# daniloceano/LorenzCycleToolkit

Measured on NVIDIA B200. Metric: LEC timesteps/s (all terms), 0.25°×37-lvl ERA5 shape; % of HBM roofline, higher is better.
Workload: dtype f32

## Files before the change

### lorenzcycletoolkit_b200/csrc/lec_row_body.inc

```
#if LEC_BODY_EDGE == 2
    const bool edge_iter = (it == 0) || (it == niter - 1) || (VEC == 1);
#else
    constexpr bool edge_iter = (LEC_BODY_EDGE != 0);
#endif
    if (!edge_iter || lane_on) {
    CT wgv[VEC], cav[VEC], ccv[VEC];
#pragma unroll
    for (int e = 0; e < VEC; ++e) { wgv[e] = CT(1); cav[e] = cxa_u; ccv[e] = cxc_u; }
    if constexpr (LONW >= 1) {
      if constexpr (sizeof(CT) == 4) {
        float w4[VEC];
        LEC_TAB_LOAD(LEC_TAB_WL + col, w4);
#pragma unroll
        for (int e = 0; e < VEC; ++e) wgv[e] = CT(w4[e]);
        if constexpr (LONW == 2) {
          float a4[VEC], c4[VEC];
          LEC_TAB_LOAD(LEC_TAB_CXA + col, a4);
          LEC_TAB_LOAD(LEC_TAB_CXC + col, c4);
#pragma unroll
          for (int e = 0; e < VEC; ++e) { cav[e] = rc.fx * CT(a4[e]); ccv[e] = rc.fx * CT(c4[e]); }
        }
      } else {
#pragma unroll
        for (int e = 0; e < VEC; ++e) {
// ... 48 lines not shown
        const P tc = P::make(CT(Tc[e]), CT(Tc[e + 1]));
        const P dtdt = pfma(P::bcast(rc.ct_m), P::make(CT(Tm[e]), CT(Tm[e + 1])) - tc,
                            pfma(P::bcast(rc.ct_p), P::make(CT(Tp[e]), CT(Tp[e + 1])) - tc, P::bcast(rc.ct_s) * tc));
        const P dTx = pfma(P::make(cav[e], cav[e + 1]), P::make(CT(tlv[e]), CT(tlv[e + 1])) - tc,
                           P::make(ccv[e], ccv[e + 1]) * (P::make(CT(trv[e]), CT(trv[e + 1])) - tc));
        const P dTy = pfma(P::bcast(rc.cy_m), P::make(CT(Tjm[e]), CT(Tjm[e + 1])) - tc,
                           P::bcast(rc.cy_p) * (P::make(CT(Tjp[e]), CT(Tjp[e + 1])) - tc));
        const P Ss = pfma(P::bcast(rc.s_m), P::make(CT(Tkm[e]), CT(Tkm[e + 1])) - tc,
                          pfma(P::bcast(rc.s_p), P::make(CT(Tkp[e]), CT(Tkp[e + 1])) - tc, P::bcast(rc.s_s) * tc));
        const P u = P::make(CT(U[e]), CT(U[e + 1])), v = P::make(CT(V[e]), CT(V[e + 1])),
                om = P::make(CT(W[e]), CT(W[e + 1]));
        q[h] = pfma(u, dTx, pfma(v, dTy, pfma(om, Ss, dtdt)));
        a[h] = tc - P::bcast(cshT); b[h] = u - P::bcast(cshU); cv[h] = v - P::bcast(cshV); w[h] = om - P::bcast(cshW);
        f[h] = P::make(CT(F[e]), CT(F[e + 1])) - P::bcast(cshF);
        if (masked) {
          const CT z = CT(0);
          a[h] = P::make(inb(e) ? a[h].lo() : z, inb(e + 1) ? a[h].hi() : z);
          b[h] = P::make(inb(e) ? b[h].lo() : z, inb(e + 1) ? b[h].hi() : z);
          cv[h] = P::make(inb(e) ? cv[h].lo() : z, inb(e + 1) ? cv[h].hi() : z);
          w[h] = P::make(inb(e) ? w[h].lo() : z, inb(e + 1) ? w[h].hi() : z);
          f[h] = P::make(inb(e) ? f[h].lo() : z, inb(e + 1) ? f[h].hi() : z);
          q[h] = P::make(inb(e) ? q[h].lo() : z, inb(e + 1) ? q[h].hi() : z);
        }
        Wa[h] = a[h]; Wb[h] = b[h]; Wc[h] = cv[h]; Ww[h] = w[h]; Wf[h] = f[h]; Wq[h] = q[h];
        if (weighted) {
          const P wg = P::make(wgv[e], wgv[e + 1]);
          Wa[h] = wg * a[h]; Wb[h] = wg * b[h]; Wc[h] = wg * cv[h]; Ww[h] = wg * w[h]; Wf[h] = wg * f[h]; Wq[h] = wg * q[h];
        }
        pbb[h] = Wb[h] * b[h]; pcc[h] = Wc[h] * cv[h]; pca[h] = Wc[h] * a[h]; pwa[h] = Ww[h] * a[h];
      }
      if constexpr (NPAIR == 2) {
        auto lin = [](P x0, P x1) { const P t = x0 + x1; return t.lo() + t.hi(); };
        auto prd = [](P x0, P y0, P x1, P y1) { const P t = pfma(x1, y1, x0 * y0); return t.lo() + t.hi(); };
        lec_lin_add<CT, COMP>(S[R_A], Cc[R_A], lin(Wa[0], Wa[1])); lec_lin_add<CT, COMP>(S[R_B], Cc[R_B], lin(Wb[0], Wb[1]));
        lec_lin_add<CT, COMP>(S[R_C], Cc[R_C], lin(Wc[0], Wc[1])); lec_lin_add<CT, COMP>(S[R_W], Cc[R_W], lin(Ww[0], Ww[1]));
        lec_lin_add<CT, COMP>(S[R_F], Cc[R_F], lin(Wf[0], Wf[1])); lec_lin_add<CT, COMP>(S[R_Q], Cc[R_Q], lin(Wq[0], Wq[1]));
        S[R_AA] += prd(Wa[0], a[0], Wa[1], a[1]); S[R_BB] += lin(pbb[0], pbb[1]); S[R_CC] += lin(pcc[0], pcc[1]);
        S[R_BC] += prd(Wb[0], cv[0], Wb[1], cv[1]); S[R_CA] += lin(pca[0], pca[1]); S[R_WA] += lin(pwa[0], pwa[1]);
        S[R_WB] += prd(Ww[0], b[0], Ww[1], b[1]); S[R_WC] += prd(Ww[0], cv[0], Ww[1], cv[1]);
        S[R_WF] += prd(Ww[0], f[0], Ww[1], f[1]); S[R_QA] += prd(Wa[0], q[0], Wa[1], q[1]);
        S[R_CAA] += prd(pca[0], a[0], pca[1], a[1]); S[R_WAA] += prd(pwa[0], a[0], pwa[1], a[1]);
        S[R_BBC] += prd(pbb[0], cv[0], pbb[1], cv[1]); S[R_CCC] += prd(pcc[0], cv[0], pcc[1], cv[1]);
        S[R_BBW] += prd(pbb[0], w[0], pbb[1], w[1]); S[R_CCW] += prd(pcc[0], w[0], pcc[1], w[1]);
      } else {
#pragma unroll
        for (int h = 0; h < NPAIR; ++h) {
          accumulate_pp<CT, COMP>(S, Cc, Wa[h].lo(), Wb[h].lo(), Wc[h].lo(), Ww[h].lo(), Wf[h].lo(), Wq[h].lo(), a[h].lo(), b[h].lo(),
                            cv[h].lo(), w[h].lo(), f[h].lo(), q[h].lo(), pbb[h].lo(), pcc[h].lo(), pca[h].lo(), pwa[h].lo());
          accumulate_pp<CT, COMP>(S, Cc, Wa[h].hi(), Wb[h].hi(), Wc[h].hi(), Ww[h].hi(), Wf[h].hi(), Wq[h].hi(), a[h].hi(), b[h].hi(),
                            cv[h].hi(), w[h].hi(), f[h].hi(), q[h].hi(), pbb[h].hi(), pcc[h].hi(), pca[h].hi(), pwa[h].hi());
        }
      }
    } else {
#pragma unroll
      for (int e = 0; e < VEC; ++e) {
        const CT tc = CT(Tc[e]);
        const CT dtdt = rc.ct_m * (CT(Tm[e]) - tc) + rc.ct_p * (CT(Tp[e]) - tc) + rc.ct_s * tc;
        const CT dTx = cav[e] * (CT(tlv[e]) - tc) + ccv[e] * (CT(trv[e]) - tc);
        const CT dTy = rc.cy_m * (CT(Tjm[e]) - tc) + rc.cy_p * (CT(Tjp[e]) - tc);
        const CT Ss = rc.s_m * (CT(Tkm[e]) - tc) + rc.s_p * (CT(Tkp[e]) - tc) + rc.s_s * tc;
        const CT u = CT(U[e]), v = CT(V[e]), om = CT(W[e]);
        CT q = dtdt + u * dTx + v * dTy + om * Ss;
        CT a = tc - cshT, b = u - cshU, cv = v - cshV, w = om - cshW, f = CT(F[e]) - cshF;
        if (masked && !inb(e)) { q = CT(0); a = CT(0); b = CT(0); cv = CT(0); w = CT(0); f = CT(0); }
        const CT wg = wgv[e];
        accumulate_s<CT, COMP>(S, Cc, wg * a, wg * b, wg * cv, wg * w, wg * f, wg * q, a, b, cv, w, f, q);
      }
    }
    }
```

### lorenzcycletoolkit_b200/csrc/lec_row_moments.cuh

```cuda
#pragma once
#include "lec_common.cuh"
#include "lec_packed.cuh"

namespace lec {

#ifndef LEC_ROWS_PER_CTA
#define LEC_ROWS_PER_CTA 2
#endif
constexpr int kRowsPerCta = LEC_ROWS_PER_CTA;
constexpr int kRowThreads = kRowsPerCta * 32;

struct FastDiv {
  unsigned mul;
  unsigned shr;
  unsigned d;
  static FastDiv make(unsigned d) {
    FastDiv f;
    unsigned L = 0;
    while ((1ull << L) < d) ++L;
    f.mul = (unsigned)(((1ull << (31 + L)) / d) + 1ull);
    f.shr = 31 + L;
    f.d = d;
    return f;
  }
// ... 25 lines not shown
  const unsigned long long a0 = reinterpret_cast<unsigned long long>(p) + (unsigned long long)lo_byte;
  const unsigned long long a1 = reinterpret_cast<unsigned long long>(p) + (unsigned long long)hi_byte;
  const unsigned long long lo = (a0 + 15ULL) & ~15ULL, hi = a1 & ~15ULL;
  if (hi <= lo) return;
  const unsigned n = unsigned(hi - lo);
  asm volatile("cp.async.bulk.prefetch.L2.global [%0], %1;" ::"l"(lo), "r"(n) : "memory");
}

#ifdef LEC_NO_STREAM
#define __ldcs __ldg
#endif
template <typename FT, int VEC> struct VecLoad;
template <> struct VecLoad<float, 4> {
  static __device__ __forceinline__ void ld(const float* p, float (&v)[4]) {
    float4 t = __ldg(reinterpret_cast<const float4*>(p)); v[0] = t.x; v[1] = t.y; v[2] = t.z; v[3] = t.w; }
  static __device__ __forceinline__ void ld_stream(const float* p, float (&v)[4]) {
    float4 t = __ldcs(reinterpret_cast<const float4*>(p)); v[0] = t.x; v[1] = t.y; v[2] = t.z; v[3] = t.w; }
};
template <> struct VecLoad<double, 2> {
  static __device__ __forceinline__ void ld(const double* p, double (&v)[2]) {
    double2 t = __ldg(reinterpret_cast<const double2*>(p)); v[0] = t.x; v[1] = t.y; }
  static __device__ __forceinline__ void ld_stream(const double* p, double (&v)[2]) {
    double2 t = __ldcs(reinterpret_cast<const double2*>(p)); v[0] = t.x; v[1] = t.y; }
};
template <typename FT> struct VecLoad<FT, 1> {
  static __device__ __forceinline__ void ld(const FT* p, FT (&v)[1]) { v[0] = __ldg(p); }
  static __device__ __forceinline__ void ld_stream(const FT* p, FT (&v)[1]) { v[0] = __ldcs(p); }
};

__device__ __forceinline__ double shfl_xor_f64(double v, int m) {
  return __shfl_xor_sync(0xffffffffu, v, m);
}

template <int N>
__device__ __forceinline__ double butterfly_reduce(double (&v)[N], int lane) {
  static_assert(N <= 32, "at most one value per lane");
  double a[32];
#pragma unroll
  for (int i = 0; i < 32; ++i) a[i] = (i < N) ? v[i] : 0.0;
  int n = 32;
#pragma unroll
  for (int bit = 16; bit >= 1; bit >>= 1) {
    n >>= 1;
    const bool hi = (lane & bit) != 0;
#pragma unroll
    for (int i = 0; i < n; ++i) {
      const int live = (N + (32 / (2 * n)) - 1) / (32 / (2 * n));
      if (2 * i < live) {
        const double keep = hi ? a[2 * i + 1] : a[2 * i];
        const double send = hi ? a[2 * i] : a[2 * i + 1];
        a[i] = keep + shfl_xor_f64(send, bit);
      } else {
        a[i] = 0.0;
      }
    }
  }
  return a[0];
}

__device__ __forceinline__ int bitrev5(int x) {
  return ((x & 1) << 4) | ((x & 2) << 2) | (x & 4) | ((x & 8) >> 2) | ((x & 16) >> 4);
}

template <typename CT>
struct RowCoefS {
  CT ct_m, ct_p, ct_s;
  CT cy_m, cy_p;
  CT s_m, s_p, s_s;
  CT fx;
};

constexpr int R_NLIN = 6;

template <typename CT, bool COMP>
__device__ __forceinline__ void lec_lin_add(CT& s, CT& c, CT x) {
  if constexpr (sizeof(CT) == 4 && COMP) {
    const CT t = s + x;
    c += x - (t - s);
    s = t;
  } else {
    s += x;
  }
}

template <typename CT, bool COMP>
__device__ __forceinline__ void accumulate_s(CT (&S)[R_NSUM], CT (&Cc)[R_NLIN], CT Wa, CT Wb, CT Wc, CT Ww, CT Wf, CT Wq,
                                           CT a, CT b, CT c, CT w, CT f, CT q) {
  lec_lin_add<CT, COMP>(S[R_A], Cc[R_A], Wa); lec_lin_add<CT, COMP>(S[R_B], Cc[R_B], Wb); lec_lin_add<CT, COMP>(S[R_C], Cc[R_C], Wc);
  lec_lin_add<CT, COMP>(S[R_W], Cc[R_W], Ww); lec_lin_add<CT, COMP>(S[R_F], Cc[R_F], Wf); lec_lin_add<CT, COMP>(S[R_Q], Cc[R_Q], Wq);
// ... 18 lines not shown
}

template <typename CT, int LONW>
struct RowSetup {
  RowCoefS<CT> rc;
  CT cxa_u, cxc_u, cxW, cxE, wW, wE;
  double fxd;
  __device__ __forceinline__ void init(const RowParams& p, const StepDev* __restrict__ st, int j, int k, int j0, int j1) {
    if constexpr (sizeof(CT) == 4) {
      rc.ct_m = st->f_ct_m; rc.ct_p = st->f_ct_p; rc.ct_s = st->f_ct_s;
      rc.cy_m = (j == j0) ? 0.f : (j == j1) ? -st->f_cyN : __ldg(p.g.cya32 + j);
      rc.cy_p = (j == j1) ? 0.f : (j == j0) ? st->f_cyS : __ldg(p.g.cyc32 + j);
      rc.s_m = __ldg(p.g.sm32 + k); rc.s_p = __ldg(p.g.sp32 + k); rc.s_s = __ldg(p.g.ss32 + k);
      rc.fx = __ldg(p.g.fxj32 + j);
      fxd = 0.0;
      cxa_u = rc.fx * p.g.cxa_u32; cxc_u = rc.fx * p.g.cxc_u32;
      cxW = rc.fx * st->f_cxW; cxE = rc.fx * st->f_cxE;
      wW = (LONW == 0) ? st->f_wWn : st->f_wW; wE = (LONW == 0) ? st->f_wEn : st->f_wE;
    } else {
      rc.ct_m = st->ct_m; rc.ct_p = st->ct_p; rc.ct_s = st->ct_s;
      rc.cy_m = (j == j0) ? 0.0 : (j == j1) ? -st->cyN : p.g.cya[j];
      rc.cy_p = (j == j1) ? 0.0 : (j == j0) ? st->cyS : p.g.cyc[j];
      rc.s_m = p.g.sm[k]; rc.s_p = p.g.sp[k]; rc.s_s = p.g.ss[k];
      fxd = p.g.fxj[j];
      rc.fx = fxd;
      cxa_u = fxd * p.g.cxa_u; cxc_u = fxd * p.g.cxc_u;
      cxW = fxd * st->cxW; cxE = fxd * st->cxE;
      const double wnorm = (LONW == 0) ? 1.0 / p.g.wl_u : 1.0;
      wW = st->wW * wnorm; wE = st->wE * wnorm;
    }
  }
};

#ifndef LEC_ROW_MIN_CTAS
#define LEC_ROW_MIN_CTAS (512 / kRowThreads)
#endif
template <typename FT, typename CT, int VEC, int LONW, bool COMP>
__global__ void __launch_bounds__(kRowThreads, sizeof(CT) == 8 ? (LEC_ROW_MIN_CTAS * 3) / 4 : COMP ? (LEC_ROW_MIN_CTAS * 3) / 4 : LEC_ROW_MIN_CTAS)
lec_row_moments_kernel(const RowParams p) {
  const int warp = threadIdx.x >> 5, lane = threadIdx.x & 31;
  const unsigned bid = blockIdx.x;
  unsigned ujt, uk, us;
  const unsigned q1 = p.dv_tiles.divmod(bid, ujt);
  const unsigned q2 = p.dv_lev.divmod(q1, uk);
  const int band = int(p.dv_steps.divmod(q2, us));
  const int jt = int(ujt), k = int(uk), s = int(us);

  const StepDev* __restrict__ st = p.steps + s;
  const int i0 = st->i0, i1 = st->i1, j0 = st->j0, j1 = st->j1;
  const int jrel = (band * p.tiles_per_band + jt) * kRowsPerCta + warp;
  if (jrel > j1 - j0) return;
  const int j = j0 + jrel;
  const int nlon = p.g.nlon, nlat = p.g.nlat, nlev = p.g.nlev;

  const long long plane = (long long)nlat * nlon;
  const long long row_c = ((long long)st->slot * nlev + k) * plane + (long long)j * nlon;
  const FT* __restrict__ Tc_row = static_cast<const FT*>(p.field[0]) + row_c;
  const FT* __restrict__ U_row = static_cast<const FT*>(p.field[1]) + row_c;
  const FT* __restrict__ V_row = static_cast<const FT*>(p.field[2]) + row_c;
  const FT* __restrict__ W_row = static_cast<const FT*>(p.field[3]) + row_c;
  const FT* __restrict__ F_row = static_cast<const FT*>(p.field[4]) + row_c;
  const int d_m = int((long long)(st->slot_m - st->slot) * p.slot_stride);
  const int d_p = int((long long)(st->slot_p - st->slot) * p.slot_stride);
  const int d_km = (k > 0) ? -int(plane) : 0, d_kp = (k < nlev - 1) ? int(plane) : 0;
  const int d_jm = (j > j0) ? -nlon : 0, d_jp = (j < j1) ? nlon : 0;

// ... 17 lines not shown
#pragma unroll
  for (int n = 0; n < R_NSUM; ++n) S[n] = CT(0);
#pragma unroll
  for (int n = 0; n < R_NLIN; ++n) Cc[n] = CT(0);

  double* __restrict__ rec = p.rec + (((long long)s * nlev + k) * p.max_ny + jrel) * LEC_NREC;

  const int c0 = i0 / VEC, c1 = i1 / VEC;
  const int niter = (c1 - c0 + 32) / 32;

  auto at = [](const FT* base, int idx) -> const FT* {
    unsigned long long a;
    asm("mad.wide.s32 %0, %1, %2, %3;" : "=l"(a) : "r"(idx), "r"((int)sizeof(FT)), "l"(base));
    return reinterpret_cast<const FT*>(a);
  };
  {
    const int it = 0;
#define LEC_BODY_EDGE 1
#include "lec_row_iter_direct.inc"
#undef LEC_BODY_EDGE
  }
  for (int it = 1; it < niter - 1; ++it) {
#define LEC_BODY_EDGE 0
#include "lec_row_iter_direct.inc"
#undef LEC_BODY_EDGE
  }
  if (niter > 1) {
    const int it = niter - 1;
#define LEC_BODY_EDGE 1
#include "lec_row_iter_direct.inc"
#undef LEC_BODY_EDGE
  }

  double Sd[R_NSUM];
#pragma unroll
  for (int n = 0; n < R_NSUM; ++n) Sd[n] = double(S[n]);
  if constexpr (sizeof(CT) == 4 && COMP) {
#pragma unroll
    for (int n = 0; n < R_NLIN; ++n) Sd[n] += double(Cc[n]);
  }
  double tot = butterfly_reduce<R_NSUM>(Sd, lane);
  if (LONW == 0) tot *= p.g.wl_u;
  const int idx = bitrev5(lane);
  if (idx < R_NSUM) rec[idx] = tot;
  if (lane == 1) {
    rec[R_SH_T] = double(shT); rec[R_SH_U] = double(shU); rec[R_SH_V] = double(shV);
    rec[R_SH_W] = double(shW); rec[R_SH_F] = double(shF);
  }
}

}
```

### lorenzcycletoolkit_b200/csrc/lec_row_narrow.cuh

```cuda
#pragma once
#include "lec_common.cuh"
#include "lec_packed.cuh"
#include "lec_row_moments.cuh"

namespace lec {

constexpr int kNarrowWarps = 1;
constexpr int kNarrowThreads = kNarrowWarps * 32;

template <int N, int G>
__device__ __forceinline__ void butterfly_reduce_seg(const double (&v)[N], int gl, double (&out)[(N + G - 1) / G]) {
  constexpr int NP = ((N + G - 1) / G) * G;
  double a[NP];
#pragma unroll
  for (int i = 0; i < NP; ++i) a[i] = (i < N) ? v[i] : 0.0;
  int n = NP;
#pragma unroll
  for (int bit = G / 2; bit >= 1; bit >>= 1) {
    n >>= 1;
    const bool hi = (gl & bit) != 0;
#pragma unroll
    for (int i = 0; i < n; ++i) {
      const double keep = hi ? a[2 * i + 1] : a[2 * i];
      const double send = hi ? a[2 * i] : a[2 * i + 1];
      a[i] = keep + __shfl_xor_sync(0xffffffffu, send, bit);
    }
  }
#pragma unroll
  for (int m = 0; m < (N + G - 1) / G; ++m) out[m] = a[m];
}

template <int G>
__device__ __forceinline__ int bitrev_group(int gl) {
  int r = 0;
#pragma unroll
  for (int b = 1, o = G / 2; b < G; b <<= 1, o >>= 1) r |= (gl & b) ? o : 0;
  return r;
}

template <typename FT, typename CT, int VEC, int LONW, int G, bool COMP>
__global__ void __launch_bounds__(kNarrowThreads, (sizeof(CT) == 8 ? 384 : 512) / kNarrowThreads)
lec_row_moments_narrow_kernel(const RowParams p) {
  constexpr int RPW = 32 / G;
  const int warp = threadIdx.x >> 5, lane31 = threadIdx.x & 31;
  const int lane = lane31 & (G - 1);
  const int wr = lane31 / G;
  const unsigned bid = blockIdx.x;
  unsigned ujt, uk, us;
  const unsigned q1 = p.dv_tiles.divmod(bid, ujt);
  const unsigned q2 = p.dv_lev.divmod(q1, uk);
  const int band = int(p.dv_steps.divmod(q2, us));
  const int jt = int(ujt), k = int(uk), s = int(us);

  const StepDev* __restrict__ st = p.steps + s;
  const int i0 = st->i0, i1 = st->i1, j0 = st->j0, j1 = st->j1;
  const int jrel_first = ((band * p.tiles_per_band + jt) * kNarrowWarps + warp) * RPW;
  if (jrel_first > j1 - j0) return;
  const bool row_on = jrel_first + wr <= j1 - j0;
  const int jrel = min(jrel_first + wr, j1 - j0);
  const int j = j0 + jrel;
  const int nlon = p.g.nlon, nlat = p.g.nlat, nlev = p.g.nlev;

// ... 26 lines not shown
  const bool box_aligned = (i0 % VEC == 0) && ((i1 + 1) % VEC == 0);

  const FT shT = __ldg(Tc_row + i0), shU = __ldg(U_row + i0), shV = __ldg(V_row + i0),
           shW = __ldg(W_row + i0), shF = __ldg(F_row + i0);
  const CT cshT = CT(shT), cshU = CT(shU), cshV = CT(shV), cshW = CT(shW), cshF = CT(shF);

  CT S[R_NSUM], Cc[R_NLIN];
#pragma unroll
  for (int n = 0; n < R_NSUM; ++n) S[n] = CT(0);
#pragma unroll
  for (int n = 0; n < R_NLIN; ++n) Cc[n] = CT(0);
  double* __restrict__ rec = p.rec + (((long long)s * nlev + k) * p.max_ny + jrel) * LEC_NREC;

  const int c0 = i0 / VEC, c1 = i1 / VEC;
  const int niter = (c1 - c0 + G) / G;
  {
    const int it = 0;
#define LEC_BODY_EDGE 1
#include "lec_row_iter_narrow.inc"
#undef LEC_BODY_EDGE
  }
  for (int it = 1; it < niter - 1; ++it) {
#define LEC_BODY_EDGE 0
#include "lec_row_iter_narrow.inc"
#undef LEC_BODY_EDGE
  }
  if (niter > 1) {
    const int it = niter - 1;
#define LEC_BODY_EDGE 1
#include "lec_row_iter_narrow.inc"
#undef LEC_BODY_EDGE
  }

  double Sd[R_NSUM];
#pragma unroll
  for (int n = 0; n < R_NSUM; ++n) Sd[n] = double(S[n]);
  if constexpr (sizeof(CT) == 4 && COMP) {
#pragma unroll
    for (int n = 0; n < R_NLIN; ++n) Sd[n] += double(Cc[n]);
  }
  constexpr int NOUT = (R_NSUM + G - 1) / G;
  double tot[NOUT];
  butterfly_reduce_seg<R_NSUM, G>(Sd, lane, tot);
  if (row_on) {
    const int r = bitrev_group<G>(lane);
#pragma unroll
    for (int m = 0; m < NOUT; ++m) {
      const int idx = r + m * G;
      if (idx < R_NSUM) rec[idx] = (LONW == 0) ? tot[m] * p.g.wl_u : tot[m];
    }
    if (lane == 1) {
      rec[R_SH_T] = double(shT); rec[R_SH_U] = double(shU); rec[R_SH_V] = double(shV);
      rec[R_SH_W] = double(shW); rec[R_SH_F] = double(shF);
    }
  }
}

}
```

### lorenzcycletoolkit_b200/csrc/lec_row_tile.cuh

```cuda
#pragma once
#include <cuda.h>

#include "lec_common.cuh"
#include "lec_packed.cuh"
#include "lec_row_moments.cuh"
#include "lec_row_narrow.cuh"

namespace lec {

struct alignas(64) TmaMaps {
  CUtensorMap t_halo;
  CUtensorMap t_plain;
  CUtensorMap u, v, w, f;
};

template <typename FT, int R, int NSTG, int GL = 32>
struct TileGeom {
  static constexpr int VEC = 16 / sizeof(FT);
  static constexpr int RPW = 32 / GL;
  static constexpr int ROWS = R * RPW;
  static constexpr int C = GL * VEC;
  static constexpr int HP = C + 2 * VEC;
  static constexpr int halo_bytes = (ROWS + 2) * HP * sizeof(FT);
  static constexpr int halo_bytes_pad = (halo_bytes + 127) / 128 * 128;
  static constexpr int tile_bytes = ROWS * C * sizeof(FT);
  static constexpr int stage_bytes = halo_bytes_pad + 8 * tile_bytes;
  static constexpr int smem_bytes = NSTG * stage_bytes + 128;
  static constexpr int threads = (R + 1) * 32;
  static __host__ __device__ constexpr int tx_bytes(int rows) { return ((rows + 2) * HP + 8 * rows * C) * (int)sizeof(FT); }
};

__device__ __forceinline__ unsigned smem_u32(const void* p) { return (unsigned)__cvta_generic_to_shared(p); }
__device__ __forceinline__ void mbar_init(unsigned bar, int count) {
  asm volatile("mbarrier.init.shared::cta.b64 [%0], %1;" ::"r"(bar), "r"(count) : "memory");
}
__device__ __forceinline__ void mbar_expect_tx(unsigned bar, unsigned bytes) {
  asm volatile("mbarrier.arrive.expect_tx.shared::cta.b64 _, [%0], %1;" ::"r"(bar), "r"(bytes) : "memory");
}
__device__ __forceinline__ void mbar_arrive(unsigned bar) {
  asm volatile("mbarrier.arrive.shared::cta.b64 _, [%0];" ::"r"(bar) : "memory");
}
__device__ __forceinline__ bool mbar_try_wait(unsigned bar, unsigned parity) {
  unsigned ok;
  asm volatile(
      "{\n .reg .pred p;\n mbarrier.try_wait.parity.shared::cta.b64 p, [%1], %2;\n selp.u32 %0, 1, 0, p;\n}"
      : "=r"(ok) : "r"(bar), "r"(parity) : "memory");
  return ok != 0;
}
__device__ __forceinline__ void mbar_wait(unsigned bar, unsigned parity) {
  while (!mbar_try_wait(bar, parity)) {}
}
template <int OFF>
__device__ __forceinline__ void mbar_arrive_off(unsigned bar) {
  asm volatile("mbarrier.arrive.shared::cta.b64 _, [%0+%1];" ::"r"(bar), "n"(OFF) : "memory");
}
__device__ __forceinline__ unsigned long long l2_policy_evict_first() {
  unsigned long long pol;
  asm volatile("createpolicy.fractional.L2::evict_first.b64 %0, 1.0;" : "=l"(pol));
  return pol;
}
// ... 13 lines not shown

template <typename FT, int VEC>
__device__ __forceinline__ void lds_vec(unsigned a, FT (&v)[VEC]) {
  if constexpr (sizeof(FT) == 4) {
    asm volatile("ld.shared.v4.f32 {%0, %1, %2, %3}, [%4];" : "=f"(v[0]), "=f"(v[1]), "=f"(v[2]), "=f"(v[3]) : "r"(a));
  } else {
    asm volatile("ld.shared.v2.f64 {%0, %1}, [%2];" : "=d"(v[0]), "=d"(v[1]) : "r"(a));
  }
}
__device__ __forceinline__ float lds_one(unsigned a, float) {
  float v; asm volatile("ld.shared.f32 %0, [%1];" : "=f"(v) : "r"(a)); return v;
}
__device__ __forceinline__ double lds_one(unsigned a, double) {
  double v; asm volatile("ld.shared.f64 %0, [%1];" : "=d"(v) : "r"(a)); return v;
}

template <bool SHARED, int VEC>
__device__ __forceinline__ void tab_load(const float* ptr, float (&v)[VEC]) {
  if constexpr (SHARED && VEC == 4) {
    const float4 t = *reinterpret_cast<const float4*>(ptr); v[0] = t.x; v[1] = t.y; v[2] = t.z; v[3] = t.w;
  } else {
    VecLoad<float, VEC>::ld(ptr, v);
  }
}

template <bool SHARED, int VEC>
__device__ __forceinline__ void tab_load_tile(const float* ptr, unsigned saddr, float (&v)[VEC]) {
  if constexpr (SHARED && VEC == 4) {
    asm volatile("ld.shared.v4.f32 {%0, %1, %2, %3}, [%4];" : "=f"(v[0]), "=f"(v[1]), "=f"(v[2]), "=f"(v[3]) : "r"(saddr));
  } else {
    VecLoad<float, VEC>::ld(ptr, v);
  }
}

struct TileId { int band, s, k, jt; };
__device__ __forceinline__ TileId decode_tile(unsigned id, const RowParams& p) {
  TileId t;
  unsigned jt, k, s;
  const unsigned a = p.dv_tiles.divmod(id, jt);
  const unsigned b = p.dv_lev.divmod(a, k);
  t.band = int(p.dv_steps.divmod(b, s));
  t.jt = int(jt); t.k = int(k); t.s = int(s);
  return t;
}

template <typename FT, typename CT, int LONW, int R, int NSTG, bool COMP, bool TABS, int GL = 32, int MINB = 1>
__global__ void __launch_bounds__((R + 1) * 32, MINB)
lec_row_moments_tile_kernel(const __grid_constant__ TmaMaps maps, const RowParams p) {
  using G = TileGeom<FT, R, NSTG, GL>;
  constexpr int VEC = G::VEC, C = G::C, HP = G::HP, RPW = G::RPW;
  const int trows = (GL == 32) ? R : p.tile_rows;
  extern __shared__ __align__(1024) unsigned char smem[];
  unsigned long long* bars = reinterpret_cast<unsigned long long*>(smem + NSTG * G::stage_bytes);
  const unsigned full0 = smem_u32(bars), empty0 = smem_u32(bars + NSTG);
  const int warp = threadIdx.x >> 5, lane = threadIdx.x & 31;

  if (threadIdx.x == 0) {
    for (int i = 0; i < NSTG; ++i) { mbar_init(full0 + 8 * i, 1); mbar_init(empty0 + 8 * i, R); }
    asm volatile("fence.mbarrier_init.release.cluster;" ::: "memory");
  }
  const float* wl_tab = p.g.wl32;
  if constexpr (TABS) {
    float* wl_s = reinterpret_cast<float*>(smem + G::smem_bytes);
    for (int i = threadIdx.x; i < p.g.nlon; i += blockDim.x) wl_s[i] = __ldg(p.g.wl32 + i);
    wl_tab = wl_s;
  }
  __syncthreads();

  const int nlev = p.g.nlev;

  if (warp == R) {
    if (lane == 0) {
      int stg = 0;
      unsigned phase = 0;
      const unsigned long long pol_stream = l2_policy_evict_first();
      for (unsigned id = blockIdx.x; id < (unsigned)p.grid; id += gridDim.x) {
        const TileId t = decode_tile(id, p);
        const StepDev* __restrict__ st = p.steps + t.s;
        const int jr = (t.band * p.tiles_per_band + t.jt) * trows;
        if (jr > st->j1 - st->j0) continue;
        const int c0 = st->i0 / VEC, c1 = st->i1 / VEC;
        const int nch = (c1 - c0 + GL) / GL;
        const unsigned tx = (unsigned)G::tx_bytes(trows);
        const unsigned tile_b = (unsigned)(trows * C * (int)sizeof(FT));
        const int jt0 = st->j0 + jr;
        const int k = t.k, km = k > 0 ? k - 1 : k, kp = k < nlev - 1 ? k + 1 : k;
        const int slot = st->slot, slot_m = st->slot_m, slot_p = st->slot_p;
        int col = c0 * VEC;
        for (int ch = 0; ch < nch; ++ch, col += C) {
          mbar_wait(empty0 + 8 * stg, phase ^ 1);
          const unsigned fb = full0 + 8 * stg;
          if (p.prefetch_mode & 2) {
            mbar_arrive(fb);
            if (++stg == NSTG) { stg = 0; phase ^= 1; }
            continue;
          }
          mbar_expect_tx(fb, tx);
          const unsigned base = smem_u32(smem) + (unsigned)stg * G::stage_bytes;
          tma_load_4d(base, &maps.t_halo, fb, col - VEC, jt0 - 1, k, slot);
          unsigned d = base + G::halo_bytes_pad;
          if (p.prefetch_mode & 8) {
            tma_load_4d_hint(d, &maps.u, fb, col, jt0, k, slot, pol_stream); d += tile_b;
            tma_load_4d_hint(d, &maps.v, fb, col, jt0, k, slot, pol_stream); d += tile_b;
            tma_load_4d_hint(d, &maps.w, fb, col, jt0, k, slot, pol_stream); d += tile_b;
            tma_load_4d_hint(d, &maps.f, fb, col, jt0, k, slot, pol_stream); d += tile_b;
          } else {
            tma_load_4d(d, &maps.u, fb, col, jt0, k, slot); d += tile_b;
            tma_load_4d(d, &maps.v, fb, col, jt0, k, slot); d += tile_b;
            tma_load_4d(d, &maps.w, fb, col, jt0, k, slot); d += tile_b;
            tma_load_4d(d, &maps.f, fb, col, jt0, k, slot); d += tile_b;
          }
          tma_load_4d(d, &maps.t_plain, fb, col, jt0, k, slot_p); d += tile_b;
          tma_load_4d(d, &maps.t_plain, fb, col, jt0, k, slot_m); d += tile_b;
          tma_load_4d(d, &maps.t_plain, fb, col, jt0, km, slot); d += tile_b;
          tma_load_4d(d, &maps.t_plain, fb, col, jt0, kp, slot);
          if (++stg == NSTG) { stg = 0; phase ^= 1; }
        }
      }
    }
    return;
  }

  const unsigned sbase0 = smem_u32(smem);
  const int gl = lane & (GL - 1);
  const int rowt = warp * RPW + lane / GL;
  const unsigned off_hc = (unsigned)(((rowt + 1) * HP + VEC + gl * VEC) * sizeof(FT));
  const unsigned off_t = (unsigned)(G::halo_bytes_pad + (rowt * C + gl * VEC) * sizeof(FT));
  const unsigned kTile = (unsigned)(trows * C * (int)sizeof(FT));
  unsigned sb = sbase0, fb = full0;
  int stg = 0;
  unsigned phase = 0;
  [[maybe_unused]] unsigned wl_s32 = 0;
  if constexpr (TABS) wl_s32 = smem_u32(smem + G::smem_bytes);
  for (unsigned id = blockIdx.x; id < (unsigned)p.grid; id += gridDim.x) {
    const TileId t = decode_tile(id, p);
    const StepDev* __restrict__ st = p.steps + t.s;
    const int i0 = st->i0, i1 = st->i1, j0 = st->j0, j1 = st->j1;
    const int jrel0 = (t.band * p.tiles_per_band + t.jt) * trows;
    if (jrel0 > j1 - j0) continue;
    const bool warp_on = (warp * RPW < trows) && (jrel0 + warp * RPW <= j1 - j0) && !(p.prefetch_mode & 4);
    const bool row_on = warp_on && (rowt < trows) && (jrel0 + rowt <= j1 - j0);
    const int jrel = row_on ? jrel0 + rowt : j1 - j0;
    const int j = j0 + jrel;
    const int k = t.k;
    const int c0 = i0 / VEC, c1 = i1 / VEC;
    const int niter = (c1 - c0 + GL) / GL;

    RowSetup<CT, LONW> rs;
    rs.init(p, st, j, k, j0, j1);
    const RowCoefS<CT>& rc = rs.rc;
    const CT cxa_u = rs.cxa_u, cxc_u = rs.cxc_u, cxW = rs.cxW, cxE = rs.cxE, wW = rs.wW, wE = rs.wE;
    [[maybe_unused]] const double fxd = rs.fxd;
    const bool box_aligned = (i0 % VEC == 0) && ((i1 + 1) % VEC == 0);
    const unsigned off_hm = (j > j0) ? off_hc - (unsigned)(HP * sizeof(FT)) : off_hc;
    const unsigned off_hp = (j < j1) ? off_hc + (unsigned)(HP * sizeof(FT)) : off_hc;

    FT shT = FT(0), shU = FT(0), shV = FT(0), shW = FT(0), shF = FT(0);
    CT cshT = CT(0), cshU = CT(0), cshV = CT(0), cshW = CT(0), cshF = CT(0);
    CT S[R_NSUM], Cc[R_NLIN];
#pragma unroll
    for (int n = 0; n < R_NSUM; ++n) S[n] = CT(0);
#pragma unroll
    for (int n = 0; n < R_NLIN; ++n) Cc[n] = CT(0);
    double* __restrict__ rec = p.rec + (((long long)t.s * nlev + k) * p.max_ny + jrel) * LEC_NREC;


    {
      const int it = 0;
#define LEC_BODY_EDGE 1
#define LEC_ITER_FIRST 1
#include "lec_row_iter_tile.inc"
#undef LEC_ITER_FIRST
#undef LEC_BODY_EDGE
    }
    for (int it = 1; it < niter - 1; ++it) {
#define LEC_BODY_EDGE 0
#define LEC_ITER_FIRST 0
#include "lec_row_iter_tile.inc"
#undef LEC_ITER_FIRST
#undef LEC_BODY_EDGE
    }
    if (niter > 1) {
      const int it = niter - 1;
#define LEC_BODY_EDGE 1
#define LEC_ITER_FIRST 0
#include "lec_row_iter_tile.inc"
#undef LEC_ITER_FIRST
#undef LEC_BODY_EDGE
    }

    if (warp_on) {
      double Sd[R_NSUM];
#pragma unroll
      for (int n = 0; n < R_NSUM; ++n) Sd[n] = double(S[n]);
      if constexpr (sizeof(CT) == 4 && COMP) {
#pragma unroll
        for (int n = 0; n < R_NLIN; ++n) Sd[n] += double(Cc[n]);
      }
      if constexpr (GL == 32) {
        double tot = butterfly_reduce<R_NSUM>(Sd, lane);
        if (LONW == 0) tot *= p.g.wl_u;
        const int idx = bitrev5(lane);
        if (idx < R_NSUM) rec[idx] = tot;
      } else {
        constexpr int NOUT = (R_NSUM + GL - 1) / GL;
        double tot[NOUT];
        butterfly_reduce_seg<R_NSUM, GL>(Sd, gl, tot);
        if (row_on) {
          const int r = bitrev_group<GL>(gl);
#pragma unroll
          for (int m = 0; m < NOUT; ++m) {
            const int idx = r + m * GL;
            if (idx < R_NSUM) rec[idx] = (LONW == 0) ? tot[m] * p.g.wl_u : tot[m];
          }
        }
      }
      if (row_on && gl == 1) {
        rec[R_SH_T] = double(shT); rec[R_SH_U] = double(shU); rec[R_SH_V] = double(shV);
        rec[R_SH_W] = double(shW); rec[R_SH_F] = double(shF);
      }
    }
  }
}

}
```

Baseline: 6423.

## Move per-tile row setup to producer warp and pair float accumulations

The TMA producer warp now computes each tile's per-row setup (coefficients, halo offsets, record pointers) into a double-buffered shared-memory header guarded by new mbarriers, so consumer warps no longer redo decode and RowSetup work at every tile. Separately, the inner accumulation updates pairs of sums with paired float adds. The warp reductions also do their first butterfly step in float before widening to double when compensation is off. The costs are extra shared memory, additional barrier handshakes, and float-precision loss in the first reduction step.

After: 6515 (median of 6 runs). 1.01x the previous value.

```diff
diff --git a/lorenzcycletoolkit_b200/csrc/lec_row_body.inc b/lorenzcycletoolkit_b200/csrc/lec_row_body.inc
--- a/lorenzcycletoolkit_b200/csrc/lec_row_body.inc
+++ b/lorenzcycletoolkit_b200/csrc/lec_row_body.inc
@@ -104,16 +104,28 @@
       if constexpr (NPAIR == 2) {
         auto lin = [](P x0, P x1) { const P t = x0 + x1; return t.lo() + t.hi(); };
         auto prd = [](P x0, P y0, P x1, P y1) { const P t = pfma(x1, y1, x0 * y0); return t.lo() + t.hi(); };
-        lec_lin_add<CT, COMP>(S[R_A], Cc[R_A], lin(Wa[0], Wa[1])); lec_lin_add<CT, COMP>(S[R_B], Cc[R_B], lin(Wb[0], Wb[1]));
-        lec_lin_add<CT, COMP>(S[R_C], Cc[R_C], lin(Wc[0], Wc[1])); lec_lin_add<CT, COMP>(S[R_W], Cc[R_W], lin(Ww[0], Ww[1]));
-        lec_lin_add<CT, COMP>(S[R_F], Cc[R_F], lin(Wf[0], Wf[1])); lec_lin_add<CT, COMP>(S[R_Q], Cc[R_Q], lin(Wq[0], Wq[1]));
-        S[R_AA] += prd(Wa[0], a[0], Wa[1], a[1]); S[R_BB] += lin(pbb[0], pbb[1]); S[R_CC] += lin(pcc[0], pcc[1]);
-        S[R_BC] += prd(Wb[0], cv[0], Wb[1], cv[1]); S[R_CA] += lin(pca[0], pca[1]); S[R_WA] += lin(pwa[0], pwa[1]);
-        S[R_WB] += prd(Ww[0], b[0], Ww[1], b[1]); S[R_WC] += prd(Ww[0], cv[0], Ww[1], cv[1]);
-        S[R_WF] += prd(Ww[0], f[0], Ww[1], f[1]); S[R_QA] += prd(Wa[0], q[0], Wa[1], q[1]);
-        S[R_CAA] += prd(pca[0], a[0], pca[1], a[1]); S[R_WAA] += prd(pwa[0], a[0], pwa[1], a[1]);
-        S[R_BBC] += prd(pbb[0], cv[0], pbb[1], cv[1]); S[R_CCC] += prd(pcc[0], cv[0], pcc[1], cv[1]);
-        S[R_BBW] += prd(pbb[0], w[0], pbb[1], w[1]); S[R_CCW] += prd(pcc[0], w[0], pcc[1], w[1]);
+        auto acc = [&](int n, CT x, CT y) {
+          if constexpr (COMP) {
+            if (n < R_NLIN) {
+              lec_lin_add<CT, COMP>(S[n], Cc[n], x); lec_lin_add<CT, COMP>(S[n + 1], Cc[n + 1], y);
+              return;
+            }
+          }
+          const P t = P::make(S[n], S[n + 1]) + P::make(x, y);
+          S[n] = t.lo(); S[n + 1] = t.hi();
+        };
+        static_assert(R_B == R_A + 1 && R_W == R_C + 1 && R_Q == R_F + 1 && R_NLIN % 2 == 0 && R_NSUM % 2 == 0, "sums pair up");
+        acc(R_A, lin(Wa[0], Wa[1]), lin(Wb[0], Wb[1]));
+        acc(R_C, lin(Wc[0], Wc[1]), lin(Ww[0], Ww[1]));
+        acc(R_F, lin(Wf[0], Wf[1]), lin(Wq[0], Wq[1]));
+        acc(R_AA, prd(Wa[0], a[0], Wa[1], a[1]), lin(pbb[0], pbb[1]));
+        acc(R_CC, lin(pcc[0], pcc[1]), prd(Wb[0], cv[0], Wb[1], cv[1]));
+        acc(R_CA, lin(pca[0], pca[1]), lin(pwa[0], pwa[1]));
+        acc(R_WB, prd(Ww[0], b[0], Ww[1], b[1]), prd(Ww[0], cv[0], Ww[1], cv[1]));
+        acc(R_WF, prd(Ww[0], f[0], Ww[1], f[1]), prd(Wa[0], q[0], Wa[1], q[1]));
+        acc(R_CAA, prd(pca[0], a[0], pca[1], a[1]), prd(pwa[0], a[0], pwa[1], a[1]));
+        acc(R_BBC, prd(pbb[0], cv[0], pbb[1], cv[1]), prd(pcc[0], cv[0], pcc[1], cv[1]));
+        acc(R_BBW, prd(pbb[0], w[0], pbb[1], w[1]), prd(pcc[0], w[0], pcc[1], w[1]));
       } else {
 #pragma unroll
         for (int h = 0; h < NPAIR; ++h) {
diff --git a/lorenzcycletoolkit_b200/csrc/lec_row_moments.cuh b/lorenzcycletoolkit_b200/csrc/lec_row_moments.cuh
--- a/lorenzcycletoolkit_b200/csrc/lec_row_moments.cuh
+++ b/lorenzcycletoolkit_b200/csrc/lec_row_moments.cuh
@@ -81,20 +81,14 @@
   return __shfl_xor_sync(0xffffffffu, v, m);
 }
 
-template <int N>
-__device__ __forceinline__ double butterfly_reduce(double (&v)[N], int lane) {
-  static_assert(N <= 32, "at most one value per lane");
-  double a[32];
-#pragma unroll
-  for (int i = 0; i < 32; ++i) a[i] = (i < N) ? v[i] : 0.0;
-  int n = 32;
-#pragma unroll
-  for (int bit = 16; bit >= 1; bit >>= 1) {
-    n >>= 1;
+template <int N, int BIT>
+__device__ __forceinline__ void butterfly_steps(double (&a)[32], int lane) {
+#pragma unroll
+  for (int bit = BIT; bit >= 1; bit >>= 1) {
     const bool hi = (lane & bit) != 0;
 #pragma unroll
-    for (int i = 0; i < n; ++i) {
-      const int live = (N + (32 / (2 * n)) - 1) / (32 / (2 * n));
+    for (int i = 0; i < bit; ++i) {
+      const int live = (N + (16 / bit) - 1) / (16 / bit);
       if (2 * i < live) {
         const double keep = hi ? a[2 * i + 1] : a[2 * i];
         const double send = hi ? a[2 * i] : a[2 * i + 1];
@@ -104,6 +98,34 @@
       }
     }
   }
+}
+
+template <int N>
+__device__ __forceinline__ double butterfly_reduce(double (&v)[N], int lane) {
+  static_assert(N <= 32, "at most one value per lane");
+  double a[32];
+#pragma unroll
+  for (int i = 0; i < 32; ++i) a[i] = (i < N) ? v[i] : 0.0;
+  butterfly_steps<N, 16>(a, lane);
+  return a[0];
+}
+
+template <int N>
+__device__ __forceinline__ double butterfly_reduce(const float (&v)[N], int lane) {
+  static_assert(N <= 32, "at most one value per lane");
+  double a[32];
+  const bool hi = (lane & 16) != 0;
+#pragma unroll
+  for (int i = 0; i < 16; ++i) {
+    if (2 * i < N) {
+      const float v0 = v[2 * i], v1 = (2 * i + 1 < N) ? v[2 * i + 1] : 0.f;
+      const float keep = hi ? v1 : v0, send = hi ? v0 : v1;
+      a[i] = double(keep) + double(__shfl_xor_sync(0xffffffffu, send, 16));
+    } else {
+      a[i] = 0.0;
+    }
+  }
+  butterfly_steps<N, 8>(a, lane);
   return a[0];
 }
 
@@ -188,6 +210,22 @@
   }
 };
 
+template <typename CT, bool COMP>
+__device__ __forceinline__ double row_reduce(const CT (&S)[R_NSUM], const CT (&Cc)[R_NLIN], int lane) {
+  if constexpr (sizeof(CT) == 4 && !COMP) {
+    return butterfly_reduce<R_NSUM>(S, lane);
+  } else {
+    double Sd[R_NSUM];
+#pragma unroll
+    for (int n = 0; n < R_NSUM; ++n) Sd[n] = double(S[n]);
+    if constexpr (sizeof(CT) == 4) {
+#pragma unroll
+      for (int n = 0; n < R_NLIN; ++n) Sd[n] += double(Cc[n]);
+    }
+    return butterfly_reduce<R_NSUM>(Sd, lane);
+  }
+}
+
 #ifndef LEC_ROW_MIN_CTAS
 #define LEC_ROW_MIN_CTAS (512 / kRowThreads)
 #endif
@@ -271,14 +309,7 @@
 #undef LEC_BODY_EDGE
   }
 
-  double Sd[R_NSUM];
-#pragma unroll
-  for (int n = 0; n < R_NSUM; ++n) Sd[n] = double(S[n]);
-  if constexpr (sizeof(CT) == 4 && COMP) {
-#pragma unroll
-    for (int n = 0; n < R_NLIN; ++n) Sd[n] += double(Cc[n]);
-  }
-  double tot = butterfly_reduce<R_NSUM>(Sd, lane);
+  double tot = row_reduce<CT, COMP>(S, Cc, lane);
   if (LONW == 0) tot *= p.g.wl_u;
   const int idx = bitrev5(lane);
   if (idx < R_NSUM) rec[idx] = tot;
diff --git a/lorenzcycletoolkit_b200/csrc/lec_row_narrow.cuh b/lorenzcycletoolkit_b200/csrc/lec_row_narrow.cuh
--- a/lorenzcycletoolkit_b200/csrc/lec_row_narrow.cuh
+++ b/lorenzcycletoolkit_b200/csrc/lec_row_narrow.cuh
@@ -8,15 +8,22 @@
 constexpr int kNarrowWarps = 1;
 constexpr int kNarrowThreads = kNarrowWarps * 32;
 
-template <int N, int G>
-__device__ __forceinline__ void butterfly_reduce_seg(const double (&v)[N], int gl, double (&out)[(N + G - 1) / G]) {
+template <int N, int G, typename T>
+__device__ __forceinline__ void butterfly_reduce_seg(const T (&v)[N], int gl, double (&out)[(N + G - 1) / G]) {
   constexpr int NP = ((N + G - 1) / G) * G;
-  double a[NP];
+  double a[NP / 2];
+  {
+    const bool hi = (gl & (G / 2)) != 0;
 #pragma unroll
-  for (int i = 0; i < NP; ++i) a[i] = (i < N) ? v[i] : 0.0;
-  int n = NP;
+    for (int i = 0; i < NP / 2; ++i) {
+      const T v0 = (2 * i < N) ? v[2 * i] : T(0), v1 = (2 * i + 1 < N) ? v[2 * i + 1] : T(0);
+      const T keep = hi ? v1 : v0, send = hi ? v0 : v1;
+      a[i] = double(keep) + double(__shfl_xor_sync(0xffffffffu, send, G / 2));
+    }
+  }
+  int n = NP / 2;
 #pragma unroll
-  for (int bit = G / 2; bit >= 1; bit >>= 1) {
+  for (int bit = G / 4; bit >= 1; bit >>= 1) {
     n >>= 1;
     const bool hi = (gl & bit) != 0;
 #pragma unroll
@@ -28,6 +35,23 @@
   }
 #pragma unroll
   for (int m = 0; m < (N + G - 1) / G; ++m) out[m] = a[m];
+}
+
+template <typename CT, bool COMP, int G>
+__device__ __forceinline__ void row_reduce_seg(const CT (&S)[R_NSUM], const CT (&Cc)[R_NLIN], int gl,
+                                               double (&out)[(R_NSUM + G - 1) / G]) {
+  if constexpr (sizeof(CT) == 4 && !COMP) {
+    butterfly_reduce_seg<R_NSUM, G>(S, gl, out);
+  } else {
+    double Sd[R_NSUM];
+#pragma unroll
+    for (int n = 0; n < R_NSUM; ++n) Sd[n] = double(S[n]);
+    if constexpr (sizeof(CT) == 4) {
+#pragma unroll
+      for (int n = 0; n < R_NLIN; ++n) Sd[n] += double(Cc[n]);
+    }
+    butterfly_reduce_seg<R_NSUM, G>(Sd, gl, out);
+  }
 }
 
 template <int G>
@@ -120,16 +144,9 @@
 #undef LEC_BODY_EDGE
   }
 
-  double Sd[R_NSUM];
-#pragma unroll
-  for (int n = 0; n < R_NSUM; ++n) Sd[n] = double(S[n]);
-  if constexpr (sizeof(CT) == 4 && COMP) {
-#pragma unroll
-    for (int n = 0; n < R_NLIN; ++n) Sd[n] += double(Cc[n]);
-  }
   constexpr int NOUT = (R_NSUM + G - 1) / G;
   double tot[NOUT];
-  butterfly_reduce_seg<R_NSUM, G>(Sd, lane, tot);
+  row_reduce_seg<CT, COMP, G>(S, Cc, lane, tot);
   if (row_on) {
     const int r = bitrev_group<G>(lane);
 #pragma unroll
diff --git a/lorenzcycletoolkit_b200/csrc/lec_row_tile.cuh b/lorenzcycletoolkit_b200/csrc/lec_row_tile.cuh
--- a/lorenzcycletoolkit_b200/csrc/lec_row_tile.cuh
+++ b/lorenzcycletoolkit_b200/csrc/lec_row_tile.cuh
@@ -25,7 +25,12 @@
   static constexpr int halo_bytes_pad = (halo_bytes + 127) / 128 * 128;
   static constexpr int tile_bytes = ROWS * C * sizeof(FT);
   static constexpr int stage_bytes = halo_bytes_pad + 8 * tile_bytes;
-  static constexpr int smem_bytes = NSTG * stage_bytes + 128;
+  static constexpr int NHDR = 2, HDR_ROW_BYTES = 160;
+  static constexpr int hdr_slot_bytes = (32 + ROWS * HDR_ROW_BYTES + 127) / 128 * 128;
+  static constexpr int hdr_off = NSTG * stage_bytes;
+  static constexpr int bar_off = hdr_off + NHDR * hdr_slot_bytes;
+  static constexpr int smem_bytes = bar_off + 128;
+  static_assert((2 * NSTG + 2 * NHDR) * 8 <= 128, "barriers fit their 128 bytes");
   static constexpr int threads = (R + 1) * 32;
   static __host__ __device__ constexpr int tx_bytes(int rows) { return ((rows + 2) * HP + 8 * rows * C) * (int)sizeof(FT); }
 };
@@ -105,6 +110,24 @@
     VecLoad<float, VEC>::ld(ptr, v);
   }
 }
+
+template <typename CT, int LONW>
+struct alignas(16) TileRowHdr {
+  RowSetup<CT, LONW> rs;
+  int jrel;
+  int live;
+  int dhm, dhp;
+};
+struct TileHdrCommon {
+  long long rec_row0;
+  int i0, i1, c0, c1, niter, box_aligned;
+  int end;
+};
+template <typename CT, int LONW, int ROWS>
+struct TileHeader {
+  TileHdrCommon t;
+  TileRowHdr<CT, LONW> row[ROWS];
+};
 
 struct TileId { int band, s, k, jt; };
 __device__ __forceinline__ TileId decode_tile(unsigned id, const RowParams& p) {
@@ -124,12 +147,17 @@
   constexpr int VEC = G::VEC, C = G::C, HP = G::HP, RPW = G::RPW;
   const int trows = (GL == 32) ? R : p.tile_rows;
   extern __shared__ __align__(1024) unsigned char smem[];
-  unsigned long long* bars = reinterpret_cast<unsigned long long*>(smem + NSTG * G::stage_bytes);
+  using Hdr = TileHeader<CT, LONW, G::ROWS>;
+  static_assert(sizeof(Hdr) <= G::hdr_slot_bytes, "tile header fits its slot");
+  unsigned long long* bars = reinterpret_cast<unsigned long long*>(smem + G::bar_off);
   const unsigned full0 = smem_u32(bars), empty0 = smem_u32(bars + NSTG);
+  const unsigned hfull0 = smem_u32(bars + 2 * NSTG), hempty0 = smem_u32(bars + 2 * NSTG + G::NHDR);
+  auto hdr = [&](int h) { return reinterpret_cast<Hdr*>(smem + G::hdr_off + h * G::hdr_slot_bytes); };
   const int warp = threadIdx.x >> 5, lane = threadIdx.x & 31;
 
   if (threadIdx.x == 0) {
     for (int i = 0; i < NSTG; ++i) { mbar_init(full0 + 8 * i, 1); mbar_init(empty0 + 8 * i, R); }
+    for (int i = 0; i < G::NHDR; ++i) { mbar_init(hfull0 + 8 * i, 1); mbar_init(hempty0 + 8 * i, R); }
     asm volatile("fence.mbarrier_init.release.cluster;" ::: "memory");
   }
   const float* wl_tab = p.g.wl32;
@@ -143,53 +171,81 @@
   const int nlev = p.g.nlev;
 
   if (warp == R) {
+    int stg = 0, hs = 0;
+    unsigned phase = 0, hphase = 0;
+    const unsigned long long pol_stream = l2_policy_evict_first();
+    for (unsigned id = blockIdx.x; id < (unsigned)p.grid; id += gridDim.x) {
+      const TileId t = decode_tile(id, p);
+      const StepDev* __restrict__ st = p.steps + t.s;
+      const int i0 = st->i0, i1 = st->i1, j0 = st->j0, j1 = st->j1;
+      const int jr = (t.band * p.tiles_per_band + t.jt) * trows;
+      if (jr > j1 - j0) continue;
+      const int k = t.k;
+      const int c0 = i0 / VEC, c1 = i1 / VEC;
+      const int nch = (c1 - c0 + GL) / GL;
+      mbar_wait(hempty0 + 8 * hs, hphase ^ 1);
+      Hdr* h = hdr(hs);
+      for (int r = lane; r < G::ROWS; r += 32) {
+        TileRowHdr<CT, LONW>& rh = h->row[r];
+        const bool live = (r < trows) && (jr + r <= j1 - j0);
+        const int jrel = live ? jr + r : j1 - j0;
+        const int j = j0 + jrel;
+        rh.rs.init(p, st, j, k, j0, j1);
+        rh.jrel = jrel;
+        rh.live = live;
+        rh.dhm = (j > j0) ? -int(HP * sizeof(FT)) : 0;
+        rh.dhp = (j < j1) ? int(HP * sizeof(FT)) : 0;
+      }
+      if (lane == 0) {
+        h->t.rec_row0 = ((long long)t.s * nlev + k) * p.max_ny;
+        h->t.i0 = i0; h->t.i1 = i1; h->t.c0 = c0; h->t.c1 = c1; h->t.niter = nch;
+        h->t.box_aligned = (i0 % VEC == 0) && ((i1 + 1) % VEC == 0);
+        h->t.end = 0;
+      }
+      __syncwarp();
+      if (lane == 0) mbar_arrive(hfull0 + 8 * hs);
+      if (++hs == G::NHDR) { hs = 0; hphase ^= 1; }
+      if (lane != 0) continue;
+      const unsigned tx = (unsigned)G::tx_bytes(trows);
+      const unsigned tile_b = (unsigned)(trows * C * (int)sizeof(FT));
+      const int jt0 = j0 + jr;
+      const int km = k > 0 ? k - 1 : k, kp = k < nlev - 1 ? k + 1 : k;
+      const int slot = st->slot, slot_m = st->slot_m, slot_p = st->slot_p;
+      int col = c0 * VEC;
+      for (int ch = 0; ch < nch; ++ch, col += C) {
+        mbar_wait(empty0 + 8 * stg, phase ^ 1);
+        const unsigned fb = full0 + 8 * stg;
+        if (p.prefetch_mode & 2) {
+          mbar_arrive(fb);
+          if (++stg == NSTG) { stg = 0; phase ^= 1; }
+          continue;
+        }
+        mbar_expect_tx(fb, tx);
+        const unsigned base = smem_u32(smem) + (unsigned)stg * G::stage_bytes;
+        tma_load_4d(base, &maps.t_halo, fb, col - VEC, jt0 - 1, k, slot);
+        unsigned d = base + G::halo_bytes_pad;
+        if (p.prefetch_mode & 8) {
+          tma_load_4d_hint(d, &maps.u, fb, col, jt0, k, slot, pol_stream); d += tile_b;
+          tma_load_4d_hint(d, &maps.v, fb, col, jt0, k, slot, pol_stream); d += tile_b;
+          tma_load_4d_hint(d, &maps.w, fb, col, jt0, k, slot, pol_stream); d += tile_b;
+          tma_load_4d_hint(d, &maps.f, fb, col, jt0, k, slot, pol_stream); d += tile_b;
+        } else {
+          tma_load_4d(d, &maps.u, fb, col, jt0, k, slot); d += tile_b;
+          tma_load_4d(d, &maps.v, fb, col, jt0, k, slot); d += tile_b;
+          tma_load_4d(d, &maps.w, fb, col, jt0, k, slot); d += tile_b;
+          tma_load_4d(d, &maps.f, fb, col, jt0, k, slot); d += tile_b;
+        }
+        tma_load_4d(d, &maps.t_plain, fb, col, jt0, k, slot_p); d += tile_b;
+        tma_load_4d(d, &maps.t_plain, fb, col, jt0, k, slot_m); d += tile_b;
+        tma_load_4d(d, &maps.t_plain, fb, col, jt0, km, slot); d += tile_b;
+        tma_load_4d(d, &maps.t_plain, fb, col, jt0, kp, slot);
+        if (++stg == NSTG) { stg = 0; phase ^= 1; }
+      }
+    }
+    mbar_wait(hempty0 + 8 * hs, hphase ^ 1);
     if (lane == 0) {
-      int stg = 0;
-      unsigned phase = 0;
-      const unsigned long long pol_stream = l2_policy_evict_first();
-      for (unsigned id = blockIdx.x; id < (unsigned)p.grid; id += gridDim.x) {
-        const TileId t = decode_tile(id, p);
-        const StepDev* __restrict__ st = p.steps + t.s;
-        const int jr = (t.band * p.tiles_per_band + t.jt) * trows;
-        if (jr > st->j1 - st->j0) continue;
-        const int c0 = st->i0 / VEC, c1 = st->i1 / VEC;
-        const int nch = (c1 - c0 + GL) / GL;
-        const unsigned tx = (unsigned)G::tx_bytes(trows);
-        const unsigned tile_b = (unsigned)(trows * C * (int)sizeof(FT));
-        const int jt0 = st->j0 + jr;
-        const int k = t.k, km = k > 0 ? k - 1 : k, kp = k < nlev - 1 ? k + 1 : k;
-        const int slot = st->slot, slot_m = st->slot_m, slot_p = st->slot_p;
-        int col = c0 * VEC;
-        for (int ch = 0; ch < nch; ++ch, col += C) {
-          mbar_wait(empty0 + 8 * stg, phase ^ 1);
-          const unsigned fb = full0 + 8 * stg;
-          if (p.prefetch_mode & 2) {
-            mbar_arrive(fb);
-            if (++stg == NSTG) { stg = 0; phase ^= 1; }
-            continue;
-          }
-          mbar_expect_tx(fb, tx);
-          const unsigned base = smem_u32(smem) + (unsigned)stg * G::stage_bytes;
-          tma_load_4d(base, &maps.t_halo, fb, col - VEC, jt0 - 1, k, slot);
-          unsigned d = base + G::halo_bytes_pad;
-          if (p.prefetch_mode & 8) {
-            tma_load_4d_hint(d, &maps.u, fb, col, jt0, k, slot, pol_stream); d += tile_b;
-            tma_load_4d_hint(d, &maps.v, fb, col, jt0, k, slot, pol_stream); d += tile_b;
-            tma_load_4d_hint(d, &maps.w, fb, col, jt0, k, slot, pol_stream); d += tile_b;
-            tma_load_4d_hint(d, &maps.f, fb, col, jt0, k, slot, pol_stream); d += tile_b;
-          } else {
-            tma_load_4d(d, &maps.u, fb, col, jt0, k, slot); d += tile_b;
-            tma_load_4d(d, &maps.v, fb, col, jt0, k, slot); d += tile_b;
-            tma_load_4d(d, &maps.w, fb, col, jt0, k, slot); d += tile_b;
-            tma_load_4d(d, &maps.f, fb, col, jt0, k, slot); d += tile_b;
-          }
-          tma_load_4d(d, &maps.t_plain, fb, col, jt0, k, slot_p); d += tile_b;
-          tma_load_4d(d, &maps.t_plain, fb, col, jt0, k, slot_m); d += tile_b;
-          tma_load_4d(d, &maps.t_plain, fb, col, jt0, km, slot); d += tile_b;
-          tma_load_4d(d, &maps.t_plain, fb, col, jt0, kp, slot);
-          if (++stg == NSTG) { stg = 0; phase ^= 1; }
-        }
-      }
+      hdr(hs)->t.end = 1;
+      mbar_arrive(hfull0 + 8 * hs);
     }
     return;
   }
@@ -205,28 +261,24 @@
   unsigned phase = 0;
   [[maybe_unused]] unsigned wl_s32 = 0;
   if constexpr (TABS) wl_s32 = smem_u32(smem + G::smem_bytes);
-  for (unsigned id = blockIdx.x; id < (unsigned)p.grid; id += gridDim.x) {
-    const TileId t = decode_tile(id, p);
-    const StepDev* __restrict__ st = p.steps + t.s;
-    const int i0 = st->i0, i1 = st->i1, j0 = st->j0, j1 = st->j1;
-    const int jrel0 = (t.band * p.tiles_per_band + t.jt) * trows;
-    if (jrel0 > j1 - j0) continue;
-    const bool warp_on = (warp * RPW < trows) && (jrel0 + warp * RPW <= j1 - j0) && !(p.prefetch_mode & 4);
-    const bool row_on = warp_on && (rowt < trows) && (jrel0 + rowt <= j1 - j0);
-    const int jrel = row_on ? jrel0 + rowt : j1 - j0;
-    const int j = j0 + jrel;
-    const int k = t.k;
-    const int c0 = i0 / VEC, c1 = i1 / VEC;
-    const int niter = (c1 - c0 + GL) / GL;
-
-    RowSetup<CT, LONW> rs;
-    rs.init(p, st, j, k, j0, j1);
+  int hs = 0;
+  unsigned hphase = 0;
+  for (;;) {
+    mbar_wait(hfull0 + 8 * hs, hphase);
+    const Hdr* h = hdr(hs);
+    if (h->t.end) break;
+    const int i0 = h->t.i0, i1 = h->t.i1, c0 = h->t.c0, c1 = h->t.c1, niter = h->t.niter;
+    const bool box_aligned = h->t.box_aligned != 0;
+    const bool warp_on = h->row[warp * RPW].live && !(p.prefetch_mode & 4);
+    const TileRowHdr<CT, LONW>& rh = h->row[rowt];
+    const bool row_on = warp_on && rh.live;
+
+    const RowSetup<CT, LONW> rs = rh.rs;
     const RowCoefS<CT>& rc = rs.rc;
     const CT cxa_u = rs.cxa_u, cxc_u = rs.cxc_u, cxW = rs.cxW, cxE = rs.cxE, wW = rs.wW, wE = rs.wE;
     [[maybe_unused]] const double fxd = rs.fxd;
-    const bool box_aligned = (i0 % VEC == 0) && ((i1 + 1) % VEC == 0);
-    const unsigned off_hm = (j > j0) ? off_hc - (unsigned)(HP * sizeof(FT)) : off_hc;
-    const unsigned off_hp = (j < j1) ? off_hc + (unsigned)(HP * sizeof(FT)) : off_hc;
+    const unsigned off_hm = off_hc + (unsigned)rh.dhm, off_hp = off_hc + (unsigned)rh.dhp;
+    double* __restrict__ rec = p.rec + (h->t.rec_row0 + rh.jrel) * LEC_NREC;
 
     FT shT = FT(0), shU = FT(0), shV = FT(0), shW = FT(0), shF = FT(0);
     CT cshT = CT(0), cshU = CT(0), cshV = CT(0), cshW = CT(0), cshF = CT(0);
@@ -235,8 +287,6 @@
     for (int n = 0; n < R_NSUM; ++n) S[n] = CT(0);
 #pragma unroll
     for (int n = 0; n < R_NLIN; ++n) Cc[n] = CT(0);
-    double* __restrict__ rec = p.rec + (((long long)t.s * nlev + k) * p.max_ny + jrel) * LEC_NREC;
-
 
     {
       const int it = 0;
@@ -263,22 +313,15 @@
     }
 
     if (warp_on) {
-      double Sd[R_NSUM];
-#pragma unroll
-      for (int n = 0; n < R_NSUM; ++n) Sd[n] = double(S[n]);
-      if constexpr (sizeof(CT) == 4 && COMP) {
-#pragma unroll
-        for (int n = 0; n < R_NLIN; ++n) Sd[n] += double(Cc[n]);
-      }
       if constexpr (GL == 32) {
-        double tot = butterfly_reduce<R_NSUM>(Sd, lane);
+        double tot = row_reduce<CT, COMP>(S, Cc, lane);
         if (LONW == 0) tot *= p.g.wl_u;
         const int idx = bitrev5(lane);
         if (idx < R_NSUM) rec[idx] = tot;
       } else {
         constexpr int NOUT = (R_NSUM + GL - 1) / GL;
         double tot[NOUT];
-        butterfly_reduce_seg<R_NSUM, GL>(Sd, gl, tot);
+        row_reduce_seg<CT, COMP, GL>(S, Cc, gl, tot);
         if (row_on) {
           const int r = bitrev_group<GL>(gl);
 #pragma unroll
@@ -293,7 +336,10 @@
         rec[R_SH_W] = double(shW); rec[R_SH_F] = double(shF);
       }
     }
-  }
-}
-
-}
+    __syncwarp();
+    if (lane == 0) mbar_arrive(hempty0 + 8 * hs);
+    if (++hs == G::NHDR) { hs = 0; hphase ^= 1; }
+  }
+}
+
+}
```
